# manhofer/Line3Dpp

Measured on AMD Instinct MI355X. Metric: M segment-pair scores/sec, higher is better.
Workload: dtype f64

## Files before the change

line3dpp_amd/csrc/k_lists.hip:

```cpp
#include <algorithm>
#include <cstdlib>
#include <type_traits>

#include "l3d_dev.h"
#include "l3d_kernels.h"
#include "l3d_lists.h"

constexpr uint32_t kLists4Grid = 512;

namespace l3d {

namespace {

#define L3D_LDS __attribute__((address_space(3)))

__device__ __forceinline__ uint32_t lane_id() { return threadIdx.x & 63u; }

template <int WPL>
__device__ __forceinline__ void group_barrier() {
    if (WPL == 1) {
        __builtin_amdgcn_fence(__ATOMIC_RELEASE, "wavefront");
        __builtin_amdgcn_wave_barrier();
        __builtin_amdgcn_fence(__ATOMIC_ACQUIRE, "wavefront");
    } else {
// ... 728 lines not shown
                lp.cands[w++] = r;
            });
        }
        if (t == 0) lp.chdrs[pool * lp.scap + hb] = CandHdr{g, c0, H, 0u};
    }
}

__global__ __launch_bounds__(256) __attribute__((amdgpu_waves_per_eu(4))) void k_cand_exact(
        const ViewDev* __restrict__ views, const PairDesc* __restrict__ pairs, const uint32_t* __restrict__ gseg_view,
        const SimConst sc, const ListPools lp) {
    if (lp.flags[0] | lp.flags[2]) return;
    const uint32_t pool = lp.pool0 + blockIdx.y, x = blockIdx.x * 256 + threadIdx.x;
    if (x >= min(lp.cnt[pool * 16 + 3], lp.ccap)) return;
    CandRec* cr = lp.cands + (size_t)pool * lp.ccap + x;
    const CandRec r = *cr;
    const uint32_t g = __float_as_uint(r.sim);
    const PairDesc& pd = pairs[r.pf_i & 0x7FFFFFFFu];
    const uint32_t tvi = (r.pf_i & kHypInv) ? pd.src : pd.tgt;
    float sim = -1.0f;
    const bool ok = exact_support(views[gseg_view[g]], views, views[0].segx[g], r.a1, r.a2, tvi, r.b1, r.b2, sc, sim);
    cr->sim = ok ? sim : -1.0f;
}

constexpr uint32_t kEdgeLds = 512;
__device__ __forceinline__ void edges_of_segment(const PairDesc* __restrict__ pairs, const Slot* __restrict__ slots,
                                                 const ListPools& lp, uint32_t* __restrict__ seg_of_g, const CandHdr ch,
                                                 uint32_t opool, L3D_LDS uint32_t* s_ij_w, L3D_LDS float* s_sim_w,
                                                 uint32_t lane) {
    const uint32_t g = ch.g, n = ch.cnt;
    CandRec* cand = lp.cands + ch.begin;
    const uint64_t lt_mask = (1ull << lane) - 1ull;
    const bool in_lds = n <= kEdgeLds;
    uint32_t n_acc = 0;
    for (uint32_t x0 = 0; x0 < n; x0 += 64) {
        const uint32_t x = x0 + lane;
        bool ok = false;
        if (x < n) {
            const float sim = cand[x].sim;
            ok = sim >= 0.0f;
            if (in_lds) { s_ij_w[x] = cand[x].ij; s_sim_w[x] = sim; }
        }
        n_acc += (uint32_t)__popcll(__builtin_amdgcn_ballot_w64(ok));
    }
    if (n_acc == 0) return;
    if (in_lds) {
        __builtin_amdgcn_fence(__ATOMIC_RELEASE, "workgroup");
        __builtin_amdgcn_wave_barrier();
        __builtin_amdgcn_fence(__ATOMIC_ACQUIRE, "workgroup");
    } else if (lane == 0) {
        atomicAdd(&lp.flags[kFlagEdgesGlobal], 1u);
    }
    auto ij_of = [&](uint32_t y) -> uint32_t { return in_lds ? s_ij_w[y] : cand[y].ij; };
    auto sim_of = [&](uint32_t y) -> float { return in_lds ? s_sim_w[y] : cand[y].sim; };
    auto in_run = [&](uint32_t x, uint32_t& rank, uint32_t& earlier, uint32_t& mine) {
        const uint32_t ij = ij_of(x), i = ij >> 16;
        rank = 0; earlier = 0; mine = 1;
        for (uint32_t y = x; y-- > 0;) {
            const uint32_t o = ij_of(y);
            if ((o >> 16) != i) break;
            if (sim_of(y) >= 0.0f) { ++earlier; ++mine; rank += o < ij ? 1u : 0u; }
        }
        for (uint32_t y = x + 1; y < n; ++y) {
            const uint32_t o = ij_of(y);
            if ((o >> 16) != i) break;
            if (sim_of(y) >= 0.0f) { ++mine; rank += o < ij ? 1u : 0u; }
        }
    };
    uint32_t n_h = 0;
    for (uint32_t x0 = 0; x0 < n; x0 += 64) {
        const uint32_t x = x0 + lane;
        bool first = false;
        if (x < n && sim_of(x) >= 0.0f) {
            const uint32_t i = ij_of(x) >> 16;
            first = true;
            for (uint32_t y = x; y-- > 0;) {
                if ((ij_of(y) >> 16) != i) break;
                if (sim_of(y) >= 0.0f) { first = false; break; }
            }
        }
        n_h += (uint32_t)__popcll(__builtin_amdgcn_ballot_w64(first));
    }
    uint32_t eb = 0, hb = 0, sb = 0;
    if (lane == 0) {
        eb = atomicAdd(&lp.cnt[opool * 16 + 0], n_acc);
        hb = atomicAdd(&lp.cnt[opool * 16 + 1], n_h);
        sb = atomicAdd(&lp.cnt[opool * 16 + 2], 1u);
    }
    eb = __shfl(eb, 0); hb = __shfl(hb, 0); sb = __shfl(sb, 0);
    if (eb + n_acc > lp.ecap || hb + n_h > lp.hcap || sb + 1 > lp.scap) {
        if (lane == 0) atomicOr(&lp.flags[0], 1u);
        return;
    }
    const uint32_t e0 = opool * lp.ecap + eb, h0 = opool * lp.hcap + hb;
    uint32_t acc_before = 0, first_before = 0;
    for (uint32_t x0 = 0; x0 < n; x0 += 64) {
        const uint32_t x = x0 + lane;
        bool acc = false, first = false;
        uint32_t rank = 0, earlier = 0, mine = 0;
        float sim = -1.0f;
        if (x < n) {
            sim = sim_of(x);
            acc = sim >= 0.0f;
            if (acc) { in_run(x, rank, earlier, mine); first = earlier == 0; }
        }
        const uint64_t ma = __builtin_amdgcn_ballot_w64(acc), mf = __builtin_amdgcn_ballot_w64(first);
        if (acc) {
            const CandRec r = cand[x];
            const uint32_t run0 = acc_before + (uint32_t)__popcll(ma & lt_mask) - earlier;
            EdgeRec e;
            e.ref_j = r.ref_j; e.sim = sim;
            e.j_cam = (r.ij & 0xFFFFu) | ((r.tvj & kHypInv) ? kEdgeInv : 0u);
            e.tv_j = r.tvj & 0x7FFFFFFFu;
            lp.edges[e0 + run0 + rank] = e;
            if (first) {
                HypHdr hdr;
                hdr.g = g; hdr.ref = r.ref_i; hdr.pair_flags = r.pf_i; hdr.canon = r.ij >> 16;
                hdr.dp1 = r.a1; hdr.dp2 = r.a2;
                hdr.edge_begin = e0 + run0; hdr.edge_cnt = mine; hdr.score3D = 0.0f; hdr.state = 0;
                {
                    const Slot hs = slots[r.ref_i];
                    const bool hinv = (r.pf_i & kHypInv) != 0;
                    const PairDesc& hp = pairs[r.pf_i & 0x7FFFFFFFu];
                    hdr.tgt_seg = !hinv ? hs.tgt_seg : lp.slot_row ? lp.slot_row[r.ref_i] : (uint32_t)((r.ref_i - hp.slot_off) / hp.K);
                    hdr.overlap = hs.overlap;
                    hdr.oq1 = hinv ? hs.dp1 : hs.dq1; hdr.oq2 = hinv ? hs.dp2 : hs.dq2;
                }
                hdr.pad[0] = hdr.pad[1] = 0;
                lp.hyps[h0 + first_before + (uint32_t)__popcll(mf & lt_mask)] = hdr;
            }
        }
        acc_before += (uint32_t)__popcll(ma); first_before += (uint32_t)__popcll(mf);
    }
    if (lane == 0) {
        const uint32_t si = opool * lp.scap + sb;
        lp.segs[si] = SegHdr{g, h0, n_h, 0u};
        seg_of_g[g] = si;
    }
}

constexpr uint32_t kEdgesSplit = 4;
__global__ __launch_bounds__(64) void k_edges(const ViewDev* __restrict__ views, const PairDesc* __restrict__ pairs,
                                               const uint32_t* __restrict__ gseg_view, const Slot* __restrict__ slots,
                                               const ListPools lp, uint32_t* __restrict__ seg_of_g) {
    const uint32_t pool = lp.pool0 + blockIdx.y, lane = lane_id();
    if (lp.flags[0] | lp.flags[2]) return;
    __shared__ uint32_t s_ij[kEdgeLds];
    __shared__ float s_sim[kEdgeLds];
    const uint32_t n_hdr = min(lp.cnt[pool * 16 + 4], lp.scap);
    for (uint32_t k = blockIdx.x; k < n_hdr; k += gridDim.x) {
        const uint32_t opool = lp.pool0 + (k + 61u * blockIdx.y) % lp.npools;
        edges_of_segment(pairs, slots, lp, seg_of_g, lp.chdrs[pool * lp.scap + k], opool, (L3D_LDS uint32_t*)s_ij, (L3D_LDS float*)s_sim, lane);
        __builtin_amdgcn_fence(__ATOMIC_RELEASE, "workgroup");
        __builtin_amdgcn_wave_barrier();
    }
}

__global__ void k_chain_sweep(const ListPools lp, uint8_t* __restrict__ positive, uint32_t* __restrict__ changed,
                              uint32_t* __restrict__ undecided) {
    if (lp.flags[0] | lp.flags[2]) return;
    const uint32_t pool = lp.pool0 + blockIdx.y, k = blockIdx.x * blockDim.x + threadIdx.x;
    bool later = false;
    if (k < min(lp.cnt[pool * 16 + 1], lp.hcap)) {
        const HypHdr& h = lp.hyps[pool * lp.hcap + k];
        if (!(h.pair_flags & kHypInv) && !__hip_atomic_load(&positive[h.ref], __ATOMIC_RELAXED, __HIP_MEMORY_SCOPE_AGENT)) {
            const uint32_t n = h.edge_cnt, e0 = h.edge_begin;
            bool done = false, any_inverse = false;
            for (uint32_t e = 0; e < n && !done; ++e) {
                const EdgeRec& ed = lp.edges[e0 + e];
                const bool inv = (ed.j_cam & kEdgeInv) != 0;
                any_inverse |= inv;
                if (!inv || __hip_atomic_load(&positive[ed.ref_j], __ATOMIC_RELAXED, __HIP_MEMORY_SCOPE_AGENT)) {
                    __hip_atomic_store(&positive[h.ref], (uint8_t)1, __ATOMIC_RELAXED, __HIP_MEMORY_SCOPE_AGENT);
                    changed[0] = 1;
                    done = true;
                }
            }
            later = !done && any_inverse;
        }
    }
    const uint64_t m = __builtin_amdgcn_ballot_w64(later);
    if (m) {
        uint32_t base = 0;
        if ((threadIdx.x & 63u) == (uint32_t)__builtin_ctzll(m)) base = atomicAdd(&lp.cnt[pool * 16 + 7], (uint32_t)__popcll(m));
        base = __shfl(base, __builtin_ctzll(m));
        if (later) undecided[pool * lp.hcap + base + (uint32_t)__popcll(m & ((1ull << (threadIdx.x & 63u)) - 1ull))] = pool * lp.hcap + k;
    }
}
constexpr uint32_t kChainListBlocks = 4;
__global__ void k_chain_sweep_list(const ListPools lp, uint8_t* __restrict__ positive, uint32_t* __restrict__ changed,
                                   uint32_t sweep, const uint32_t* __restrict__ undecided) {
    if (lp.flags[0] | lp.flags[2]) return;
    if (!changed[sweep - 1]) return;
    const uint32_t pool = lp.pool0 + blockIdx.y;
    const uint32_t n_u = min(lp.cnt[pool * 16 + 7], lp.hcap);
    for (uint32_t idx = blockIdx.x * blockDim.x + threadIdx.x; idx < n_u; idx += gridDim.x * blockDim.x) {
        const HypHdr& h = lp.hyps[undecided[pool * lp.hcap + idx]];
        if (__hip_atomic_load(&positive[h.ref], __ATOMIC_RELAXED, __HIP_MEMORY_SCOPE_AGENT)) continue;
        const uint32_t n = h.edge_cnt, e0 = h.edge_begin;
        for (uint32_t e = 0; e < n; ++e) {
            const EdgeRec& ed = lp.edges[e0 + e];
            if ((ed.j_cam & kEdgeInv) && __hip_atomic_load(&positive[ed.ref_j], __ATOMIC_RELAXED, __HIP_MEMORY_SCOPE_AGENT)) {
                __hip_atomic_store(&positive[h.ref], (uint8_t)1, __ATOMIC_RELAXED, __HIP_MEMORY_SCOPE_AGENT);
                changed[sweep] = 1;
                break;
            }
        }
    }
}

constexpr uint32_t kMaxReplicas = 16;
__global__ void k_hyp_scores(const ListPools lp, const uint8_t* __restrict__ positive,
                             const uint32_t* __restrict__ gseg_view, Slot* __restrict__ slots,
                             const uint8_t* __restrict__ pair_present, uint32_t* __restrict__ max_score_bits) {
    const uint32_t pool = lp.pool0 + blockIdx.y, k = blockIdx.x * blockDim.x + threadIdx.x;
    const bool active = !(lp.flags[0] | lp.flags[2]) && k < min(lp.cnt[pool * 16 + 1], lp.hcap);
    float score3D = 0.0f;
    uint32_t view = kEmpty;
    if (active) {
        HypHdr& h = lp.hyps[pool * lp.hcap + k];
        const bool inv = (h.pair_flags & kHypInv) != 0;
        const bool exists = !inv || positive[h.ref] != 0;
        float cur = 0.0f;
        uint32_t cur_cam = kEmpty;
        if (exists) {
            const uint32_t n = h.edge_cnt, e0 = h.edge_begin;
            for (uint32_t e = 0; e < n; e += 4) {
                EdgeRec ed[4]; bool ok[4];
#pragma unroll
                for (uint32_t i = 0; i < 4; ++i) ed[i] = lp.edges[e0 + min(e + i, n - 1)];
#pragma unroll
                for (uint32_t i = 0; i < 4; ++i) ok[i] = e + i < n && (!(ed[i].j_cam & kEdgeInv) || positive[ed[i].ref_j] != 0);
#pragma unroll
                for (uint32_t i = 0; i < 4; ++i) {
                    if (!ok[i]) continue;
                    if (ed[i].tv_j == cur_cam) {
                        if (ed[i].sim > cur) { score3D -= cur; score3D += ed[i].sim; cur = ed[i].sim; }
                    } else {
                        score3D += ed[i].sim; cur = ed[i].sim; cur_cam = ed[i].tv_j;
                    }
                }
            }
        }
        h.score3D = score3D;
        h.state = exists ? kHypExists : 0u;
        if (exists && !inv && (!pair_present || pair_present[h.pair_flags & 0x7FFFFFFFu])) slots[h.ref].score3D = score3D;
        view = gseg_view[h.g];
    }
    uint64_t todo = __builtin_amdgcn_ballot_w64(score3D > 0.0f);
    while (todo) {
        const uint32_t leader = (uint32_t)__builtin_ctzll(todo);
        const uint32_t lv = __builtin_amdgcn_readlane(view, leader);
        const bool mine = score3D > 0.0f && view == lv;
        float mx = mine ? score3D : 0.0f;
#pragma unroll
        for (int d = 32; d > 0; d >>= 1) mx = fmaxf(mx, __shfl_xor(mx, d));
        if (lane_id() == leader) {
            uint32_t* p = &max_score_bits[lv * kMaxReplicas + (pool & (kMaxReplicas - 1))];
            if (__float_as_uint(mx) > *(volatile uint32_t*)p) atomicMax(p, __float_as_uint(mx));
        }
        todo &= ~__builtin_amdgcn_ballot_w64(mine);
    }
}

__global__ void k_hyp_filter(const ListPools lp, const uint32_t* __restrict__ gseg_view,
                             const uint32_t* __restrict__ max_score_bits, uint32_t* __restrict__ kept_cnt,
                             unsigned long long* __restrict__ best_pack) {
    const uint32_t pool = lp.pool0 + blockIdx.y, k = blockIdx.x * blockDim.x + threadIdx.x;
    if ((lp.flags[0] | lp.flags[2]) || k >= min(lp.cnt[pool * 16 + 1], lp.hcap)) return;
    HypHdr& h = lp.hyps[pool * lp.hcap + k];
    uint32_t mx = 0;
    {
        const uint32_t* p = max_score_bits + (size_t)gseg_view[h.g] * kMaxReplicas;
#pragma unroll
        for (uint32_t r = 0; r < kMaxReplicas; ++r) mx = max(mx, p[r]);
    }
    const float lim = kMinBestScorePerc * __uint_as_float(mx);
    const float s = h.score3D;
    if ((h.state & kHypExists) && s > 0.0f && s > lim) {
        h.state |= kHypKeep;
        atomicAdd(&kept_cnt[h.g], 1u);
        atomicMax(&best_pack[h.g], ((unsigned long long)__float_as_uint(s) << 32) | (0xFFFFFFFFu - h.canon));
    }
}

// ... 160 lines not shown
            const uint32_t n = nv - a < 65535u ? nv - a : 65535u;                                                          \
            hipLaunchKernelGGL((k_lists<1, B>), dim3(max_M, n), dim3(64), lds1, st, views, pairs, lviews, opairs, ipairs,  \
                               gseg_view, poff, inv, hyp_p, hyp_q, uniform_K, lp, v0 + a);                                        \
        }                                                                                                                  \
           \
        hipLaunchKernelGGL((k_lists<2, B>), dim3(kLists2Grid), dim3(128), lds2, st, views, pairs, lviews, opairs, ipairs, \
                           gseg_view, poff, inv, hyp_p, hyp_q, uniform_K, lp, 0u);                                                \
            \
            \
        if (hsa.run_tier4)                                                                                                 \
        hipLaunchKernelGGL((k_lists<4, B>), dim3(kLists4Grid), dim3(256), lds4, st, views, pairs, lviews, opairs, ipairs, \
                           gseg_view, poff, inv, hyp_p, hyp_q, uniform_K, lp, 0u);                                                \
    } while (0)
    if (wide) L3D_LISTS(256); else L3D_LISTS(128);
#undef L3D_LISTS
    HugeScratch hs;
    hs.d1 = hsa.f32; hs.d2 = hsa.f32 + hsa.cap;
    hs.tv = hsa.u32; hs.ref = hsa.u32 + hsa.cap; hs.pf = hsa.u32 + 2 * (size_t)hsa.cap;
    hs.key = hsa.u64; hs.cap = hsa.cap;
    if (hsa.run_huge)
        hipLaunchKernelGGL(k_lists_huge, dim3(256), dim3(256), 0, st, views, pairs, lviews, opairs, ipairs, gseg_view, poff,
                           inv, hyp_p, hyp_q, lp, hs);
    hipLaunchKernelGGL(k_cand_exact, dim3((lp.ccap + 255) / 256, lp.npools), dim3(256), 0, st, views, pairs, gseg_view, sc, lp);
    hipLaunchKernelGGL(k_edges, dim3((lp.scap + kEdgesSplit - 1) / kEdgesSplit, lp.npools), dim3(64), 0, st, views, pairs,
                       gseg_view, slots, lp, seg_of_g);
    if (lp.npools < kListPools) hipLaunchKernelGGL(k_publish_flags, dim3(1), dim3(64), 0, st, lp);
    return hipGetLastError();
}

static dim3 hyp_grid(const ListPools& lp) { return dim3((lp.hcap + 255) / 256, lp.npools); }

hipError_t launch_chain_sweep(ListPools lp, uint8_t* positive, uint32_t* changed, uint32_t sweep, uint32_t* undecided, hipStream_t st) {
    if (sweep == 0) hipLaunchKernelGGL(k_chain_sweep, hyp_grid(lp), dim3(256), 0, st, lp, positive, changed, undecided);
    else hipLaunchKernelGGL(k_chain_sweep_list, dim3(kChainListBlocks, lp.npools), dim3(256), 0, st, lp, positive, changed, sweep, undecided);
    return hipGetLastError();
}
hipError_t launch_hyp_scores(ListPools lp, const uint8_t* positive, const uint32_t* gseg_view, Slot* slots,
                             const uint8_t* pair_present, uint32_t* max_score_bits, hipStream_t st) {
    hipLaunchKernelGGL(k_hyp_scores, hyp_grid(lp), dim3(256), 0, st, lp, positive, gseg_view, slots, pair_present, max_score_bits);
    return hipGetLastError();
}
hipError_t launch_hyp_filter(ListPools lp, uint32_t g0, uint32_t g1, const uint32_t* gseg_view, const uint32_t* max_score_bits,
                             uint32_t* kept_cnt, unsigned long long* best_pack, unsigned long long* cnt64,
                             hipStream_t st) {
    hipLaunchKernelGGL(k_hyp_filter, hyp_grid(lp), dim3(256), 0, st, lp, gseg_view, max_score_bits, kept_cnt, best_pack);
    if (g1 > g0) hipLaunchKernelGGL(k_seg_filter, dim3((g1 - g0 + 255) / 256), dim3(256), 0, st, g0, g1, kept_cnt, best_pack, cnt64);
    return hipGetLastError();
}
// ... 23 lines not shown
```

line3dpp_amd/csrc/l3d_kernels.h:

```cpp
#pragma once
#include <atomic>

#include "l3d_dev.h"

struct l3d_cledge;

namespace l3d {

extern std::atomic<uint64_t> g_knn_replay_calls;
extern std::atomic<uint64_t> g_keep_all_repeats;
extern std::atomic<uint64_t> g_live_blocks[2];
extern std::atomic<uint64_t> g_csr_global_launches;
enum ListCounter : uint32_t { kLcTier2Lists = 0, kLcTier4Lists, kLcHugeLists, kLcWidePasses, kLcNarrowPasses, kLcTierRepeats,
                              kLcHugeScratchRegrows, kLcEdgesGlobalSegments, kLcCandPoolRegrows, kLcEdgePoolRegrows, kLcCount };
extern std::atomic<uint64_t> g_list_counters[kLcCount];
extern const char* const kListCounterNames[kLcCount];
extern std::atomic<uint64_t> g_seam_support_lists[4];
extern std::atomic<uint64_t> g_seam_score_unstaged_lists;
enum SupportTier : uint32_t { kSupportNone = 0, kSupportWave, kSupportGroupStaged, kSupportSortOnly, kSupportAllPairs };
struct ListTier { SupportTier support; bool score_unstaged; };
ListTier list_tier(uint32_t L);

constexpr int kMatchRows = 64;
constexpr uint32_t kTileClasses = 5;
constexpr uint32_t kTileMinItems = 24;
__host__ __device__ constexpr uint32_t tile_classes(uint32_t Ms, uint32_t R) { return Ms / R < kTileMinItems ? 2u : kTileClasses; }
__host__ __device__ constexpr uint32_t tile_src_cap(uint32_t Ms, uint32_t R) {
    return ((Ms + tile_classes(Ms, R) * (R - 1) + R - 1) / R) * R;
}
constexpr uint64_t kMatchTileMaxItems = 2048;
uint32_t match_tile_rows(int mode, bool brute, uint64_t est_row_items);
uint32_t match_layout_rows(int mode, bool brute, uint32_t tile_rows);
struct WorkItem {
    uint32_t pair;
    uint32_t src0;
};

// ... 64 lines not shown
                              uint32_t* row_counts, float thr, CullPools pools, OrientFuse of, bool ix16,
                              uint32_t tile_rows, hipStream_t stream);
uint32_t match_tied_grid(uint32_t scratch_stride);
hipError_t launch_queue_all_rows(const PairDesc* pairs, uint32_t first, uint32_t count, uint32_t max_Ms, uint32_t list_base,
                                 OrientFuse of, hipStream_t stream);
hipError_t launch_match_tied_rows(const ViewDev* views, const PairDesc* pairs, Slot* slots, uint32_t maxK, float thr,
                                  OrientFuse of, CullPools cp, uint64_t* scratch, uint32_t scratch_stride,
                                  hipStream_t stream);
hipError_t launch_pack_slot_idx(const Slot* slots, uint32_t* idx, uint64_t lo, uint64_t hi, hipStream_t stream);
hipError_t launch_expand_slot_idx(const ViewDev* views, const PairDesc* pairs, uint32_t first, uint32_t count,
                                  uint32_t max_row_slots, const uint32_t* idx, Slot* slots, OrientFuse of,
                                  hipStream_t stream);
constexpr uint32_t kKeepBlock = 1024;
hipError_t launch_keep_pair_info(const PairDesc* pairs, uint32_t n_pairs, const uint32_t* row_counts, const uint32_t* row_start,
                                 uint4* info, uint32_t* row_pair, uint32_t* blk_row, uint32_t n_blk, uint32_t* longest, hipStream_t stream);
hipError_t launch_keep_assemble(const ViewDev* views, const PairDesc* pairs, uint32_t n_rows, uint64_t slot_cap, const uint32_t* row_start,
                                const uint32_t* row_pair, const uint32_t* blk_row, const uint32_t* longest, Slot* slots, OrientFuse of,
                                hipStream_t stream);
hipError_t launch_prep_views(const ViewDev* views, uint32_t n_views, uint32_t max_M, hipStream_t stream);

struct InvRec; struct ListPools; struct PairCsr;
constexpr uint32_t kWideMeanList = 96;
constexpr uint32_t kFlagEdgesGlobal = 8;
struct HugeScratchArgs { float* f32; uint32_t* u32; uint64_t* u64; uint32_t cap; uint32_t mean_list; uint32_t run_huge; uint32_t run_tier4; };
hipError_t launch_scan64(const unsigned long long* in, uint32_t n, unsigned long long* out, unsigned long long* tmp,
                         unsigned long long* total, hipStream_t st);
hipError_t launch_pair_csr(const PairDesc* pairs, uint32_t n_pairs, uint32_t max_Mt, const PairCsr* pair_csr,
                           const uint32_t* inv_tgt, uint32_t tgt16, uint32_t* poff, uint32_t* refs,
                           uint32_t* dummy, uint32_t tgt_v0, uint32_t tgt_v1, uint64_t max_pair_slots,
                           const uint32_t* row_start, hipStream_t st);
hipError_t launch_seg_index(ListPools lp, uint32_t* seg_of_g, uint32_t G, uint32_t world, hipStream_t st);
struct ListView; struct OutPair; struct InPair;
hipError_t launch_lists(uint32_t v0, uint32_t nv, uint32_t max_M, const ViewDev* views, const PairDesc* pairs,
                        const ListView* lviews, const OutPair* opairs, const InPair* ipairs, const uint32_t* gseg_view,
                        const uint32_t* poff, const uint32_t* inv_refs, const float2* hyp_p, const float2* hyp_q,
                        const Slot* slots, uint32_t uniform_K,
                        SimConst sc, ListPools lp, uint32_t* seg_of_g, HugeScratchArgs hsa, hipStream_t st);
hipError_t launch_chain_sweep(ListPools lp, uint8_t* positive, uint32_t* changed, uint32_t sweep, uint32_t* undecided,
                              hipStream_t st);
hipError_t launch_hyp_scores(ListPools lp, const uint8_t* positive, const uint32_t* gseg_view, Slot* slots,
                             const uint8_t* pair_present, uint32_t* max_score_bits, hipStream_t st);
hipError_t launch_hyp_filter(ListPools lp, uint32_t g0, uint32_t g1, const uint32_t* gseg_view, const uint32_t* max_score_bits,
                             uint32_t* kept_cnt, unsigned long long* best_pack, unsigned long long* cnt64,
                             hipStream_t st);
hipError_t launch_seg_write(uint32_t g0, uint32_t g1, unsigned long long base64, const ViewDev* views, const PairDesc* pairs, const uint32_t* seg_base,
                            const uint32_t* gseg_view, const unsigned long long* off64s,
                            const unsigned long long* best_pack, const uint32_t* seg_of_g, ListPools lp,
// ... 62 lines not shown
```

line3dpp_amd/csrc/l3d_phase_b.hip:

```cpp
#include "l3d_ctx.h"

namespace l3d {
std::atomic<uint64_t> g_list_counters[kLcCount];
const char* const kListCounterNames[kLcCount] = {"lists_tier2_lists", "lists_tier4_lists", "lists_huge_lists", "lists_wide_passes",
                                                 "lists_narrow_passes", "lists_tier_repeats", "lists_huge_scratch_regrows",
                                                 "edges_global_segments", "lists_cand_pool_regrows", "lists_edge_pool_regrows"};
}

extern "C" {

static int match_finish_impl(l3d_ctx* c);
static int lists_prepare(l3d_ctx* c, int caps_mode);
static int lists_reserve(l3d_ctx* c);
static int lists_run(l3d_ctx* c, uint32_t v0, uint32_t nv, uint32_t pool0, uint32_t npools);

static int lists_shard_impl(l3d_ctx* c, uint32_t rank, uint32_t world, int64_t view0, int64_t view1, void* slab_ptr[4],
                            uint64_t slab_bytes[4], void* full_ptr[4]) {
    if (!c || !slab_ptr || !slab_bytes || !full_ptr) return fail(L3D_ERR_ARG, "null argument");
    std::lock_guard<std::recursive_mutex> lk(c->mu);
    if (c->state != l3d_ctx::BEGUN) return fail(L3D_ERR_STATE, "l3d_match_begin must precede l3d_lists_shard");
    (void)hipSetDevice(c->device);
    const int rc = [&]() -> int {
        if (world == 0 || world > kListPools || rank >= world) return fail(L3D_ERR_ARG, "rank / world out of range");
        const uint32_t V = (uint32_t)c->order.size();
        uint32_t v0, v1;
        if (view0 >= 0) {
            if (view1 < view0 || (uint64_t)view1 > V) return fail(L3D_ERR_ARG, "view range out of bounds");
            v0 = (uint32_t)view0; v1 = (uint32_t)view1;
        } else {
// ... 266 lines not shown
    const ZeroLayout z = zero_layout(V, G);
    const ListPools lp = list_pools(c, pool0, npools);
    const SimConst simc = sim_thresholds(c->two_sigA_sqr);
    uint64_t max_slots = 0;
    for (uint32_t p = 0; p < P; ++p) max_slots = std::max<uint64_t>(max_slots, c->pair_slots(p));
    L3D_HIP_CHECK(hipMemsetAsync(c->d_lzero.p, 0, z.words * 4 + std::max<uint64_t>(c->n_slots, 1), st));
    g_trace.mark("zero block memset enqueued");
    const ListView* lviews = (const ListView*)c->d_ltab.p;
    const OutPair* opairs = (const OutPair*)(c->d_ltab.p + (size_t)V * 32);
    const InPair* ipairs = (const InPair*)(c->d_ltab.p + ((size_t)V + P) * 32);
    const PairCsr* pair_poff = (const PairCsr*)(c->d_ltab.p + ((size_t)V + P) * 32 + (size_t)c->n_in_pairs * 16);
    {
        uint32_t max_Mt = 0;
        for (auto& pd : c->pairs) if (pd.tgt > pd.src && pd.tgt >= v0 && pd.tgt < v0 + nv) max_Mt = std::max(max_Mt, pd.Mt);
        if (max_Mt) {
            if (max_Mt > 32768 || std::getenv("L3D_CSR_GLOBAL")) L3D_HIP_CHECK(c->d_csr_dummy.reserve((size_t)P * 64));
            L3D_HIP_CHECK(launch_pair_csr(c->d_pairs.p, P, max_Mt, pair_poff, c->d_inv_tgt.p, c->tgt16, c->d_poff.p, c->d_inv_refs.p,
                                          c->d_csr_dummy.p, v0, v0 + nv, max_slots, c->ragged ? c->d_row_start.p : nullptr, st));
        }
    }
    g_trace.mark("pair CSRs enqueued");
    const uint32_t mean_list = c->n_ents ? (uint32_t)(c->n_ents / std::max<uint32_t>(G, 1))
                                         : (uint32_t)(1.5 * (double)c->n_slots / std::max<uint32_t>(G, 1));
    const HugeScratchArgs hsa{c->d_huge_f32.p, c->d_huge_u32.p, (uint64_t*)c->d_huge_u64.p, c->huge_cap, mean_list,
                              c->huge_skip ? 0u : 1u, c->list4_skip ? 0u : 1u};
    c->huge_ran = !c->huge_skip; c->list4_ran = !c->list4_skip;
    c->lists_wide = mean_list > kWideMeanList;
    uint32_t max_M = 0;
    for (uint32_t vi = v0; vi < v0 + nv; ++vi) max_M = std::max(max_M, c->order[vi]->M);
    L3D_HIP_CHECK(launch_lists(v0, nv, max_M, c->d_views.p, c->d_pairs.p, lviews, opairs, ipairs, c->d_gseg_view.p,
                               c->d_poff.p, c->d_inv_refs.p, c->d_hyp_p.p, c->d_hyp_q.p, c->d_slots.p, c->kNN > 0 ? (uint32_t)c->kNN : 0u, simc, lp,
                               c->d_seg_of_g.p, hsa, st));
    if (c->ev_on(9)) L3D_HIP_CHECK(hipEventRecord(c->ev[9], st));
    g_trace.mark("list pass enqueued");
    return L3D_OK;
}

struct TailShard { uint32_t v0, v1, g0, g1, pool0, npools; };
static TailShard whole_tail(const l3d_ctx* c) { return TailShard{0u, (uint32_t)c->order.size(), 0u, c->G, 0u, kListPools}; }

static int tail_count_run(l3d_ctx* c, bool fresh, const TailShard& ts) {
    g_trace.mark("tail_run enter");
    hipStream_t st = c->stream;
    const uint32_t V = (uint32_t)c->order.size(), G = c->G;
    const ZeroLayout z = zero_layout(V, G);
    const bool dep = ts.npools < kListPools && c->shard_world > 1 && c->shard_dep_rank0 <= c->shard_rank;
    const uint32_t cp0 = dep ? c->shard_dep_rank0 * c->shard_ppr : 0u, cp1 = dep ? (c->shard_rank + 1) * c->shard_ppr : kListPools;
    const ListPools lp = list_pools(c, cp0, cp1 - cp0), lps = list_pools(c, ts.pool0, ts.npools);
// ... 100 lines not shown
    const uint32_t V = (uint32_t)c->order.size();
    const uint32_t* h = c->h_fin.p;
    const uint32_t* h0 = h + kFinHead;
    const uint32_t* changed = h + kListPools * 16 + 32;
    c->n_surv = h0[2]; c->n_hyps = h0[3];
    c->tm.tied_rows = h0[0];
    {
        uint64_t ents = 0, inv = 0, cands = 0, hdrs = 0;
        for (uint32_t q = 0; q < kListPools; ++q) { ents += h[q * 16 + 5]; inv += h[q * 16 + 6]; cands += h[q * 16 + 3]; hdrs += h[q * 16 + 1]; }
        c->n_ents = (uint32_t)std::min<uint64_t>(ents, 0xFFFFFFFFu);
        c->tm.list_entries = c->n_ents;
        c->tm.list_inverse = (uint32_t)std::min<uint64_t>(inv, 0xFFFFFFFFu);
        c->tm.list_candidates = (uint32_t)std::min<uint64_t>(cands, 0xFFFFFFFFu);
        c->tm.list_headers = (uint32_t)std::min<uint64_t>(hdrs, 0xFFFFFFFFu);
        c->tm.slots_lo = (uint32_t)c->n_slots; c->tm.slots_hi = (uint32_t)(c->n_slots >> 32);
    }
    {
        const uint32_t* hf = h + kListPools * 16;
        g_list_counters[kLcTier2Lists].fetch_add(hf[7], std::memory_order_relaxed);
        g_list_counters[kLcTier4Lists].fetch_add(hf[4], std::memory_order_relaxed);
        g_list_counters[kLcHugeLists].fetch_add(hf[5], std::memory_order_relaxed);
        g_list_counters[c->lists_wide ? kLcWidePasses : kLcNarrowPasses].fetch_add(1, std::memory_order_relaxed);
        g_list_counters[kLcEdgesGlobalSegments].fetch_add(hf[kFlagEdgesGlobal], std::memory_order_relaxed);
    }
    for (uint32_t s2 = 0; s2 < c->chain_enqueued; ++s2) c->tm.chain_sweeps += changed[s2] ? 1u : 0u;
    c->chain_need = c->tm.chain_extra_rounds ? kChainSweeps : c->tm.chain_sweeps;
    c->chain_hist[c->chain_hist_at++ & 3u] = c->chain_need;
    {
        uint64_t ne = 0;
        uint32_t me = 0, mh = 0, ms = 0, mc = 0;
        for (uint32_t q = 0; q < kListPools; ++q) {
            ne += h[q * 16];
            me = std::max(me, h[q * 16]); mh = std::max(mh, h[q * 16 + 1]);
            ms = std::max(ms, std::max(h[q * 16 + 2], h[q * 16 + 4])); mc = std::max(mc, h[q * 16 + 3]);
        }
        c->tm.support_words = (uint32_t)ne;
        auto fit = [](uint32_t cap, uint32_t need, uint32_t lowest) {
            const uint32_t want = std::max(need + need / 4 + 64, lowest);
            return cap > want + want / 2 ? want : cap;
        };
        c->lp_ecap = fit(c->lp_ecap, me, 256); c->lp_hcap = fit(c->lp_hcap, mh, 128);
        c->lp_scap = fit(c->lp_scap, ms, 64); c->lp_ccap = fit(c->lp_ccap, mc, 512);
    }
    for (uint32_t vi = 0; vi < V; ++vi) c->order[vi]->median_depth = ((const float*)h0)[8 + vi];
    c->host_offsets_valid = false;
    if (c->timing_pending) {
// ... 188 lines not shown
```

Before: 964,400.

## Process short segments in 16-lane groups in k_edges and prefetch edges in scoring

k_edges now packs four segments per wave, one per 16-lane group with its own LDS slice, for segments up to a group cap. Longer segments fall back to a whole-wave pass, which walks the headers a second time. The grid is capped at a fixed wave count, and new counters record how many segments took each path. The chain-sweep and score kernels now load headers and edges as 128-bit vector loads, software-prefetch the next edge batch and positive bytes, and hoist the per-view max-score atomic so each lane issues at most one, skipping it when a hint read shows no increase. The aim is better lane use on short lists and lower memory latency, at the cost of more complexity, extra counter atomics, and possible divergence.

```diff
diff --git a/line3dpp_amd/csrc/k_lists.hip b/line3dpp_amd/csrc/k_lists.hip
--- a/line3dpp_amd/csrc/k_lists.hip
+++ b/line3dpp_amd/csrc/k_lists.hip
@@ -1,4 +1,5 @@
 #include <algorithm>
+#include <cstddef>
 #include <cstdlib>
 #include <type_traits>
 
@@ -774,32 +775,75 @@
     cr->sim = ok ? sim : -1.0f;
 }
 
+template <class T>
+__device__ __forceinline__ void pin1(const T& v) { asm volatile("" ::"v"(v)); }
+template <class... T>
+__device__ __forceinline__ void pin(const T&... v) { (pin1(v), ...); }
+__device__ __forceinline__ void pin(const uint4& q) { asm volatile("" ::"v"(q.x), "v"(q.y), "v"(q.z), "v"(q.w)); }
+__device__ __forceinline__ HypHdr load_hdr(const HypHdr* p) {
+    union { HypHdr h; uint4 q[4]; } u;
+    const uint4* s = reinterpret_cast<const uint4*>(p);
+    u.q[0] = s[0]; u.q[1] = s[1]; u.q[2] = s[2]; u.q[3] = s[3];
+    return u.h;
+}
+struct HypHead {
+    uint32_t g, ref, pair_flags, canon;
+    float dp1, dp2;
+    uint32_t edge_begin, edge_cnt;
+};
+__device__ __forceinline__ HypHead load_hdr_head(const HypHdr* p) {
+    static_assert(offsetof(HypHdr, edge_cnt) == 28, "the chain's fields are the header's first 32 bytes");
+    union { HypHead h; uint4 q[2]; } u;
+    const uint4* s = reinterpret_cast<const uint4*>(p);
+    u.q[0] = s[0]; u.q[1] = s[1];
+    pin(u.q[0]); pin(u.q[1]);
+    return u.h;
+}
+template <bool PIN = true>
+__device__ __forceinline__ EdgeRec load_edge(const EdgeRec* p) {
+    union { EdgeRec e; uint4 q; } u;
+    u.q = *reinterpret_cast<const uint4*>(p);
+    if (PIN) pin(u.q);
+    return u.e;
+}
 constexpr uint32_t kEdgeLds = 512;
+constexpr uint32_t kEdgeGroup = 16, kEdgeGroups = 64 / kEdgeGroup;
+constexpr uint32_t kEdgeGroupLds = kEdgeLds / kEdgeGroups;
+static_assert(kEdgesGroupCapDefault == kEdgeGroupLds, "the default border between groups and waves is what a group's LDS holds");
+template <uint32_t W>
 __device__ __forceinline__ void edges_of_segment(const PairDesc* __restrict__ pairs, const Slot* __restrict__ slots,
                                                  const ListPools& lp, uint32_t* __restrict__ seg_of_g, const CandHdr ch,
                                                  uint32_t opool, L3D_LDS uint32_t* s_ij_w, L3D_LDS float* s_sim_w,
                                                  uint32_t lane) {
+    constexpr uint32_t kLds = W == 64 ? kEdgeLds : kEdgeGroupLds;
     const uint32_t g = ch.g, n = ch.cnt;
+    const uint32_t gl = lane & (W - 1), gb = lane - gl;
     CandRec* cand = lp.cands + ch.begin;
-    const uint64_t lt_mask = (1ull << lane) - 1ull;
-    const bool in_lds = n <= kEdgeLds;
+    using Mask = std::conditional_t<W == 64, uint64_t, uint32_t>;
+    const Mask lt_mask = (Mask)(((Mask)1 << gl) - 1);
+    auto gballot = [&](bool f) -> Mask {
+        const uint64_t m = __builtin_amdgcn_ballot_w64(f);
+        return W == 64 ? (Mask)m : (Mask)((uint32_t)(m >> gb) & ((1u << (W & 31)) - 1u));
+    };
+    auto popc = [](Mask m) -> uint32_t { return W == 64 ? (uint32_t)__popcll(m) : (uint32_t)__popc((uint32_t)m); };
+    const bool in_lds = W != 64 || n <= kLds;
     uint32_t n_acc = 0;
-    for (uint32_t x0 = 0; x0 < n; x0 += 64) {
-        const uint32_t x = x0 + lane;
+    for (uint32_t x0 = 0; x0 < n; x0 += W) {
+        const uint32_t x = x0 + gl;
         bool ok = false;
         if (x < n) {
             const float sim = cand[x].sim;
             ok = sim >= 0.0f;
             if (in_lds) { s_ij_w[x] = cand[x].ij; s_sim_w[x] = sim; }
         }
-        n_acc += (uint32_t)__popcll(__builtin_amdgcn_ballot_w64(ok));
+        n_acc += popc(gballot(ok));
     }
     if (n_acc == 0) return;
     if (in_lds) {
         __builtin_amdgcn_fence(__ATOMIC_RELEASE, "workgroup");
         __builtin_amdgcn_wave_barrier();
         __builtin_amdgcn_fence(__ATOMIC_ACQUIRE, "workgroup");
-    } else if (lane == 0) {
+    } else if (gl == 0) {
         atomicAdd(&lp.flags[kFlagEdgesGlobal], 1u);
     }
     auto ij_of = [&](uint32_t y) -> uint32_t { return in_lds ? s_ij_w[y] : cand[y].ij; };
@@ -819,8 +863,8 @@
         }
     };
     uint32_t n_h = 0;
-    for (uint32_t x0 = 0; x0 < n; x0 += 64) {
-        const uint32_t x = x0 + lane;
+    for (uint32_t x0 = 0; x0 < n; x0 += W) {
+        const uint32_t x = x0 + gl;
         bool first = false;
         if (x < n && sim_of(x) >= 0.0f) {
             const uint32_t i = ij_of(x) >> 16;
@@ -830,23 +874,19 @@
                 if (sim_of(y) >= 0.0f) { first = false; break; }
             }
         }
-        n_h += (uint32_t)__popcll(__builtin_amdgcn_ballot_w64(first));
-    }
-    uint32_t eb = 0, hb = 0, sb = 0;
-    if (lane == 0) {
-        eb = atomicAdd(&lp.cnt[opool * 16 + 0], n_acc);
-        hb = atomicAdd(&lp.cnt[opool * 16 + 1], n_h);
-        sb = atomicAdd(&lp.cnt[opool * 16 + 2], 1u);
-    }
-    eb = __shfl(eb, 0); hb = __shfl(hb, 0); sb = __shfl(sb, 0);
+        n_h += popc(gballot(first));
+    }
+    uint32_t resv = 0;
+    if (gl < 3) resv = atomicAdd(&lp.cnt[opool * 16 + gl], gl == 0 ? n_acc : gl == 1 ? n_h : 1u);
+    const uint32_t eb = __shfl(resv, (int)gb), hb = __shfl(resv, (int)gb + 1), sb = __shfl(resv, (int)gb + 2);
     if (eb + n_acc > lp.ecap || hb + n_h > lp.hcap || sb + 1 > lp.scap) {
-        if (lane == 0) atomicOr(&lp.flags[0], 1u);
+        if (gl == 0) atomicOr(&lp.flags[0], 1u);
         return;
     }
     const uint32_t e0 = opool * lp.ecap + eb, h0 = opool * lp.hcap + hb;
     uint32_t acc_before = 0, first_before = 0;
-    for (uint32_t x0 = 0; x0 < n; x0 += 64) {
-        const uint32_t x = x0 + lane;
+    for (uint32_t x0 = 0; x0 < n; x0 += W) {
+        const uint32_t x = x0 + gl;
         bool acc = false, first = false;
         uint32_t rank = 0, earlier = 0, mine = 0;
         float sim = -1.0f;
@@ -855,10 +895,10 @@
             acc = sim >= 0.0f;
             if (acc) { in_run(x, rank, earlier, mine); first = earlier == 0; }
         }
-        const uint64_t ma = __builtin_amdgcn_ballot_w64(acc), mf = __builtin_amdgcn_ballot_w64(first);
+        const Mask ma = gballot(acc), mf = gballot(first);
         if (acc) {
             const CandRec r = cand[x];
-            const uint32_t run0 = acc_before + (uint32_t)__popcll(ma & lt_mask) - earlier;
+            const uint32_t run0 = acc_before + popc(ma & lt_mask) - earlier;
             EdgeRec e;
             e.ref_j = r.ref_j; e.sim = sim;
             e.j_cam = (r.ij & 0xFFFFu) | ((r.tvj & kHypInv) ? kEdgeInv : 0u);
@@ -873,38 +913,80 @@
                     const Slot hs = slots[r.ref_i];
                     const bool hinv = (r.pf_i & kHypInv) != 0;
                     const PairDesc& hp = pairs[r.pf_i & 0x7FFFFFFFu];
-                    hdr.tgt_seg = !hinv ? hs.tgt_seg : lp.slot_row ? lp.slot_row[r.ref_i] : (uint32_t)((r.ref_i - hp.slot_off) / hp.K);
+                    const uint64_t hp_off = hp.slot_off; const uint32_t hp_K = hp.K;
+                    pin(hs.tgt_seg, hs.overlap, hs.dp1, hs.dp2, hs.dq1, hs.dq2, hp_off, hp_K);
+                    hdr.tgt_seg = !hinv ? hs.tgt_seg : lp.slot_row ? lp.slot_row[r.ref_i] : (uint32_t)((r.ref_i - hp_off) / hp_K);
                     hdr.overlap = hs.overlap;
                     hdr.oq1 = hinv ? hs.dp1 : hs.dq1; hdr.oq2 = hinv ? hs.dp2 : hs.dq2;
                 }
                 hdr.pad[0] = hdr.pad[1] = 0;
-                lp.hyps[h0 + first_before + (uint32_t)__popcll(mf & lt_mask)] = hdr;
-            }
-        }
-        acc_before += (uint32_t)__popcll(ma); first_before += (uint32_t)__popcll(mf);
-    }
-    if (lane == 0) {
+                lp.hyps[h0 + first_before + popc(mf & lt_mask)] = hdr;
+            }
+        }
+        acc_before += popc(ma); first_before += popc(mf);
+    }
+    if (gl == 0) {
         const uint32_t si = opool * lp.scap + sb;
         lp.segs[si] = SegHdr{g, h0, n_h, 0u};
         seg_of_g[g] = si;
     }
 }
 
-constexpr uint32_t kEdgesSplit = 4;
-__global__ __launch_bounds__(64) void k_edges(const ViewDev* __restrict__ views, const PairDesc* __restrict__ pairs,
+#ifndef L3D_EDGES_WAVES
+#define L3D_EDGES_WAVES 8192
+#endif
+constexpr uint32_t kEdgesWaves = L3D_EDGES_WAVES;
+__global__ __launch_bounds__(64) __attribute__((amdgpu_waves_per_eu(8))) void k_edges(const ViewDev* __restrict__ views, const PairDesc* __restrict__ pairs,
                                                const uint32_t* __restrict__ gseg_view, const Slot* __restrict__ slots,
-                                               const ListPools lp, uint32_t* __restrict__ seg_of_g) {
+                                               const ListPools lp, uint32_t* __restrict__ seg_of_g, uint32_t group_cap) {
     const uint32_t pool = lp.pool0 + blockIdx.y, lane = lane_id();
+    const uint32_t gq = lane / kEdgeGroup;
+    const CandHdr* chdrs = lp.chdrs + (size_t)pool * lp.scap;
+    CandHdr ch = chdrs[min(blockIdx.x * kEdgeGroups + gq, lp.scap - 1)];
     if (lp.flags[0] | lp.flags[2]) return;
     __shared__ uint32_t s_ij[kEdgeLds];
     __shared__ float s_sim[kEdgeLds];
     const uint32_t n_hdr = min(lp.cnt[pool * 16 + 4], lp.scap);
-    for (uint32_t k = blockIdx.x; k < n_hdr; k += gridDim.x) {
-        const uint32_t opool = lp.pool0 + (k + 61u * blockIdx.y) % lp.npools;
-        edges_of_segment(pairs, slots, lp, seg_of_g, lp.chdrs[pool * lp.scap + k], opool, (L3D_LDS uint32_t*)s_ij, (L3D_LDS float*)s_sim, lane);
+    auto opool_of = [&](uint32_t k) { return lp.pool0 + (k + 61u * blockIdx.y) % lp.npools; };
+    uint32_t c_gseg = 0, c_gstep = 0, c_wseg = 0;
+    bool any_wide = false;
+    for (uint32_t k0 = blockIdx.x * kEdgeGroups; k0 < n_hdr; k0 += gridDim.x * kEdgeGroups) {
+        const uint32_t k = k0 + gq;
+        if (k0 != blockIdx.x * kEdgeGroups) ch = chdrs[min(k, lp.scap - 1)];
+        const bool valid = k < n_hdr;
+        const bool grouped = valid && group_cap != 0 && ch.cnt <= group_cap;
+        any_wide |= valid && !grouped;
+        if (grouped) {
+            edges_of_segment<kEdgeGroup>(pairs, slots, lp, seg_of_g, ch, opool_of(k), (L3D_LDS uint32_t*)s_ij + gq * kEdgeGroupLds,
+                                         (L3D_LDS float*)s_sim + gq * kEdgeGroupLds, lane);
+            if ((lane & (kEdgeGroup - 1)) == 0) { ++c_gseg; c_gstep += (ch.cnt + kEdgeGroup - 1) / kEdgeGroup; }
+        }
         __builtin_amdgcn_fence(__ATOMIC_RELEASE, "workgroup");
         __builtin_amdgcn_wave_barrier();
     }
+    if (__builtin_amdgcn_ballot_w64(any_wide)) {
+        for (uint32_t k0 = blockIdx.x * kEdgeGroups; k0 < n_hdr; k0 += gridDim.x * kEdgeGroups) {
+            const uint32_t k = k0 + gq;
+            const CandHdr wc = chdrs[min(k, lp.scap - 1)];
+            uint64_t wide = __builtin_amdgcn_ballot_w64(k < n_hdr && !(group_cap != 0 && wc.cnt <= group_cap) && (lane & (kEdgeGroup - 1)) == 0);
+            while (wide) {
+                const uint32_t src = (uint32_t)__builtin_ctzll(wide);
+                wide &= wide - 1;
+                auto from = [&](uint32_t v) { return (uint32_t)__builtin_amdgcn_readfirstlane((int)__shfl(v, (int)src)); };
+                CandHdr wh;
+                wh.g = from(wc.g); wh.begin = from(wc.begin); wh.cnt = from(wc.cnt); wh.pad = 0;
+                edges_of_segment<64>(pairs, slots, lp, seg_of_g, wh, opool_of(k0 + src / kEdgeGroup), (L3D_LDS uint32_t*)s_ij, (L3D_LDS float*)s_sim, lane);
+                ++c_wseg;
+                __builtin_amdgcn_fence(__ATOMIC_RELEASE, "workgroup");
+                __builtin_amdgcn_wave_barrier();
+            }
+        }
+    }
+    c_gseg += __shfl_xor(c_gseg, 16); c_gseg += __shfl_xor(c_gseg, 32);
+    c_gstep += __shfl_xor(c_gstep, 16); c_gstep += __shfl_xor(c_gstep, 32);
+    const uint32_t c_gstep0 = __shfl(c_gstep, 0);
+    const uint32_t c_mine = lane == 0 ? c_gseg : lane == 1 ? c_gstep0 : c_wseg;
+    if (lane < 3 && c_mine) atomicAdd(&lp.cnt[pool * 16 + kCntEdgesGroupSegs + lane], c_mine);
 }
 
 __global__ void k_chain_sweep(const ListPools lp, uint8_t* __restrict__ positive, uint32_t* __restrict__ changed,
@@ -913,12 +995,12 @@
     const uint32_t pool = lp.pool0 + blockIdx.y, k = blockIdx.x * blockDim.x + threadIdx.x;
     bool later = false;
     if (k < min(lp.cnt[pool * 16 + 1], lp.hcap)) {
-        const HypHdr& h = lp.hyps[pool * lp.hcap + k];
+        const HypHead h = load_hdr_head(lp.hyps + (size_t)pool * lp.hcap + k);
         if (!(h.pair_flags & kHypInv) && !__hip_atomic_load(&positive[h.ref], __ATOMIC_RELAXED, __HIP_MEMORY_SCOPE_AGENT)) {
             const uint32_t n = h.edge_cnt, e0 = h.edge_begin;
             bool done = false, any_inverse = false;
             for (uint32_t e = 0; e < n && !done; ++e) {
-                const EdgeRec& ed = lp.edges[e0 + e];
+                const EdgeRec ed = load_edge(lp.edges + e0 + e);
                 const bool inv = (ed.j_cam & kEdgeInv) != 0;
                 any_inverse |= inv;
                 if (!inv || __hip_atomic_load(&positive[ed.ref_j], __ATOMIC_RELAXED, __HIP_MEMORY_SCOPE_AGENT)) {
@@ -946,11 +1028,11 @@
     const uint32_t pool = lp.pool0 + blockIdx.y;
     const uint32_t n_u = min(lp.cnt[pool * 16 + 7], lp.hcap);
     for (uint32_t idx = blockIdx.x * blockDim.x + threadIdx.x; idx < n_u; idx += gridDim.x * blockDim.x) {
-        const HypHdr& h = lp.hyps[undecided[pool * lp.hcap + idx]];
+        const HypHead h = load_hdr_head(lp.hyps + undecided[pool * lp.hcap + idx]);
         if (__hip_atomic_load(&positive[h.ref], __ATOMIC_RELAXED, __HIP_MEMORY_SCOPE_AGENT)) continue;
         const uint32_t n = h.edge_cnt, e0 = h.edge_begin;
         for (uint32_t e = 0; e < n; ++e) {
-            const EdgeRec& ed = lp.edges[e0 + e];
+            const EdgeRec ed = load_edge(lp.edges + e0 + e);
             if ((ed.j_cam & kEdgeInv) && __hip_atomic_load(&positive[ed.ref_j], __ATOMIC_RELAXED, __HIP_MEMORY_SCOPE_AGENT)) {
                 __hip_atomic_store(&positive[h.ref], (uint8_t)1, __ATOMIC_RELAXED, __HIP_MEMORY_SCOPE_AGENT);
                 changed[sweep] = 1;
@@ -967,38 +1049,52 @@
     const uint32_t pool = lp.pool0 + blockIdx.y, k = blockIdx.x * blockDim.x + threadIdx.x;
     const bool active = !(lp.flags[0] | lp.flags[2]) && k < min(lp.cnt[pool * 16 + 1], lp.hcap);
     float score3D = 0.0f;
-    uint32_t view = kEmpty;
+    uint32_t view = kEmpty, hint = 0;
     if (active) {
-        HypHdr& h = lp.hyps[pool * lp.hcap + k];
+        HypHdr* hp = lp.hyps + (size_t)pool * lp.hcap + k;
+        const HypHdr h = load_hdr(hp);
         const bool inv = (h.pair_flags & kHypInv) != 0;
-        const bool exists = !inv || positive[h.ref] != 0;
+        const uint32_t n = h.edge_cnt, e0 = h.edge_begin;
+        const uint32_t e_last = e0 + (n ? n - 1 : 0);
+        EdgeRec ed[4]; uint32_t by[4];
+        auto fetch_edges = [&](uint32_t e) {
+#pragma unroll
+            for (uint32_t i = 0; i < 4; ++i) ed[i] = load_edge<false>(lp.edges + min(e0 + e + i, e_last));
+        };
+        auto fetch_bytes = [&]() {
+#pragma unroll
+            for (uint32_t i = 0; i < 4; ++i) by[i] = positive[(ed[i].j_cam & kEdgeInv) ? ed[i].ref_j : h.ref];
+        };
+        fetch_edges(0);
+        const uint32_t own = positive[h.ref];
+        const uint32_t pp = pair_present ? pair_present[h.pair_flags & 0x7FFFFFFFu] : 1u;
+        view = gseg_view[h.g];
+        fetch_bytes();
+        hint = __hip_atomic_load(&max_score_bits[view * kMaxReplicas + (pool & (kMaxReplicas - 1))], __ATOMIC_RELAXED, __HIP_MEMORY_SCOPE_AGENT);
+        const bool exists = !inv || own != 0;
         float cur = 0.0f;
         uint32_t cur_cam = kEmpty;
         if (exists) {
-            const uint32_t n = h.edge_cnt, e0 = h.edge_begin;
-            for (uint32_t e = 0; e < n; e += 4) {
-                EdgeRec ed[4]; bool ok[4];
-#pragma unroll
-                for (uint32_t i = 0; i < 4; ++i) ed[i] = lp.edges[e0 + min(e + i, n - 1)];
-#pragma unroll
-                for (uint32_t i = 0; i < 4; ++i) ok[i] = e + i < n && (!(ed[i].j_cam & kEdgeInv) || positive[ed[i].ref_j] != 0);
+            for (uint32_t e = 0; e < n;) {
 #pragma unroll
                 for (uint32_t i = 0; i < 4; ++i) {
-                    if (!ok[i]) continue;
+                    if (!(e + i < n && (!(ed[i].j_cam & kEdgeInv) || by[i] != 0))) continue;
                     if (ed[i].tv_j == cur_cam) {
                         if (ed[i].sim > cur) { score3D -= cur; score3D += ed[i].sim; cur = ed[i].sim; }
                     } else {
                         score3D += ed[i].sim; cur = ed[i].sim; cur_cam = ed[i].tv_j;
                     }
                 }
-            }
-        }
-        h.score3D = score3D;
-        h.state = exists ? kHypExists : 0u;
-        if (exists && !inv && (!pair_present || pair_present[h.pair_flags & 0x7FFFFFFFu])) slots[h.ref].score3D = score3D;
-        view = gseg_view[h.g];
+                e += 4;
+                if (e < n) { fetch_edges(e); fetch_bytes(); }
+            }
+        }
+        hp->score3D = score3D;
+        hp->state = exists ? kHypExists : 0u;
+        if (exists && !inv && pp) slots[h.ref].score3D = score3D;
     }
     uint64_t todo = __builtin_amdgcn_ballot_w64(score3D > 0.0f);
+    float lead_mx = 0.0f;
     while (todo) {
         const uint32_t leader = (uint32_t)__builtin_ctzll(todo);
         const uint32_t lv = __builtin_amdgcn_readlane(view, leader);
@@ -1006,12 +1102,11 @@
         float mx = mine ? score3D : 0.0f;
 #pragma unroll
         for (int d = 32; d > 0; d >>= 1) mx = fmaxf(mx, __shfl_xor(mx, d));
-        if (lane_id() == leader) {
-            uint32_t* p = &max_score_bits[lv * kMaxReplicas + (pool & (kMaxReplicas - 1))];
-            if (__float_as_uint(mx) > *(volatile uint32_t*)p) atomicMax(p, __float_as_uint(mx));
-        }
+        if (lane_id() == leader) lead_mx = mx;
         todo &= ~__builtin_amdgcn_ballot_w64(mine);
     }
+    if (__float_as_uint(lead_mx) > hint)
+        atomicMax(&max_score_bits[view * kMaxReplicas + (pool & (kMaxReplicas - 1))], __float_as_uint(lead_mx));
 }
 
 __global__ void k_hyp_filter(const ListPools lp, const uint32_t* __restrict__ gseg_view,
@@ -1218,8 +1313,9 @@
         hipLaunchKernelGGL(k_lists_huge, dim3(256), dim3(256), 0, st, views, pairs, lviews, opairs, ipairs, gseg_view, poff,
                            inv, hyp_p, hyp_q, lp, hs);
     hipLaunchKernelGGL(k_cand_exact, dim3((lp.ccap + 255) / 256, lp.npools), dim3(256), 0, st, views, pairs, gseg_view, sc, lp);
-    hipLaunchKernelGGL(k_edges, dim3((lp.scap + kEdgesSplit - 1) / kEdgesSplit, lp.npools), dim3(64), 0, st, views, pairs,
-                       gseg_view, slots, lp, seg_of_g);
+    const uint32_t edges_x = std::max(1u, std::min((lp.scap + kEdgeGroups - 1) / kEdgeGroups, kEdgesWaves / std::max(lp.npools, 1u)));
+    hipLaunchKernelGGL(k_edges, dim3(edges_x, lp.npools), dim3(64), 0, st, views, pairs,
+                       gseg_view, slots, lp, seg_of_g, std::min(hsa.edges_group_cap, kEdgeGroupLds));
     if (lp.npools < kListPools) hipLaunchKernelGGL(k_publish_flags, dim3(1), dim3(64), 0, st, lp);
     return hipGetLastError();
 }
diff --git a/line3dpp_amd/csrc/l3d_kernels.h b/line3dpp_amd/csrc/l3d_kernels.h
--- a/line3dpp_amd/csrc/l3d_kernels.h
+++ b/line3dpp_amd/csrc/l3d_kernels.h
@@ -12,7 +12,8 @@
 extern std::atomic<uint64_t> g_live_blocks[2];
 extern std::atomic<uint64_t> g_csr_global_launches;
 enum ListCounter : uint32_t { kLcTier2Lists = 0, kLcTier4Lists, kLcHugeLists, kLcWidePasses, kLcNarrowPasses, kLcTierRepeats,
-                              kLcHugeScratchRegrows, kLcEdgesGlobalSegments, kLcCandPoolRegrows, kLcEdgePoolRegrows, kLcCount };
+                              kLcHugeScratchRegrows, kLcEdgesGlobalSegments, kLcCandPoolRegrows, kLcEdgePoolRegrows,
+                              kLcEdgesGroupSegments, kLcEdgesGroupSteps, kLcEdgesWaveSegments, kLcCount };
 extern std::atomic<uint64_t> g_list_counters[kLcCount];
 extern const char* const kListCounterNames[kLcCount];
 extern std::atomic<uint64_t> g_seam_support_lists[4];
@@ -123,7 +124,9 @@
 struct InvRec; struct ListPools; struct PairCsr;
 constexpr uint32_t kWideMeanList = 96;
 constexpr uint32_t kFlagEdgesGlobal = 8;
-struct HugeScratchArgs { float* f32; uint32_t* u32; uint64_t* u64; uint32_t cap; uint32_t mean_list; uint32_t run_huge; uint32_t run_tier4; };
+constexpr uint32_t kCntEdgesGroupSegs = 13, kCntEdgesGroupSteps = 14, kCntEdgesWaveSegs = 15;
+constexpr uint32_t kEdgesGroupCapDefault = 128;
+struct HugeScratchArgs { float* f32; uint32_t* u32; uint64_t* u64; uint32_t cap; uint32_t mean_list; uint32_t run_huge; uint32_t run_tier4; uint32_t edges_group_cap; };
 hipError_t launch_scan64(const unsigned long long* in, uint32_t n, unsigned long long* out, unsigned long long* tmp,
                          unsigned long long* total, hipStream_t st);
 hipError_t launch_pair_csr(const PairDesc* pairs, uint32_t n_pairs, uint32_t max_Mt, const PairCsr* pair_csr,
diff --git a/line3dpp_amd/csrc/l3d_phase_b.hip b/line3dpp_amd/csrc/l3d_phase_b.hip
--- a/line3dpp_amd/csrc/l3d_phase_b.hip
+++ b/line3dpp_amd/csrc/l3d_phase_b.hip
@@ -4,7 +4,8 @@
 std::atomic<uint64_t> g_list_counters[kLcCount];
 const char* const kListCounterNames[kLcCount] = {"lists_tier2_lists", "lists_tier4_lists", "lists_huge_lists", "lists_wide_passes",
                                                  "lists_narrow_passes", "lists_tier_repeats", "lists_huge_scratch_regrows",
-                                                 "edges_global_segments", "lists_cand_pool_regrows", "lists_edge_pool_regrows"};
+                                                 "edges_global_segments", "lists_cand_pool_regrows", "lists_edge_pool_regrows",
+                                                 "edges_group_segments", "edges_group_steps", "edges_wave_segments"};
 }
 
 extern "C" {
@@ -317,8 +318,10 @@
     g_trace.mark("pair CSRs enqueued");
     const uint32_t mean_list = c->n_ents ? (uint32_t)(c->n_ents / std::max<uint32_t>(G, 1))
                                          : (uint32_t)(1.5 * (double)c->n_slots / std::max<uint32_t>(G, 1));
+    uint32_t edges_group_cap = kEdgesGroupCapDefault;
+    if (const char* e = std::getenv("L3D_EDGES_GROUP_CAP")) edges_group_cap = (uint32_t)std::min<unsigned long>(std::strtoul(e, nullptr, 10), kEdgesGroupCapDefault);
     const HugeScratchArgs hsa{c->d_huge_f32.p, c->d_huge_u32.p, (uint64_t*)c->d_huge_u64.p, c->huge_cap, mean_list,
-                              c->huge_skip ? 0u : 1u, c->list4_skip ? 0u : 1u};
+                              c->huge_skip ? 0u : 1u, c->list4_skip ? 0u : 1u, edges_group_cap};
     c->huge_ran = !c->huge_skip; c->list4_ran = !c->list4_skip;
     c->lists_wide = mean_list > kWideMeanList;
     uint32_t max_M = 0;
@@ -465,6 +468,11 @@
         g_list_counters[kLcHugeLists].fetch_add(hf[5], std::memory_order_relaxed);
         g_list_counters[c->lists_wide ? kLcWidePasses : kLcNarrowPasses].fetch_add(1, std::memory_order_relaxed);
         g_list_counters[kLcEdgesGlobalSegments].fetch_add(hf[kFlagEdgesGlobal], std::memory_order_relaxed);
+        uint64_t gs = 0, gt = 0, ws = 0;
+        for (uint32_t q = 0; q < kListPools; ++q) { gs += h[q * 16 + kCntEdgesGroupSegs]; gt += h[q * 16 + kCntEdgesGroupSteps]; ws += h[q * 16 + kCntEdgesWaveSegs]; }
+        g_list_counters[kLcEdgesGroupSegments].fetch_add(gs, std::memory_order_relaxed);
+        g_list_counters[kLcEdgesGroupSteps].fetch_add(gt, std::memory_order_relaxed);
+        g_list_counters[kLcEdgesWaveSegments].fetch_add(ws, std::memory_order_relaxed);
     }
     for (uint32_t s2 = 0; s2 < c->chain_enqueued; ++s2) c->tm.chain_sweeps += changed[s2] ? 1u : 0u;
     c->chain_need = c->tm.chain_extra_rounds ? kChainSweeps : c->tm.chain_sweeps;
```

New measurement: 1.009 million (median of 5 runs). 4.6% higher.
